# geoeo/ORB_SLAM3_V1.0

Hardware: AMD Instinct MI355X
Metric: frames/sec ORB extract+match, 752x480 8-level 1000-feat; bit-exact kp/desc (higher is better)
Workload: dtype u8

## Files before the change

### orb_slam3_v1.0_amd/csrc/kernels_match_proj.hip

```cpp
#include <algorithm>
#include <cstdio>
#include <cstdlib>
#include <cstring>

#include "device_math.h"
#include "match_common.h"

#include "match_proj.h"

#pragma clang fp contract(off)

namespace orbfe {

using namespace proj;

namespace {


template <bool LDS, class KeyFn>
__device__ __forceinline__ void block_sort_keys(unsigned long long* sKeys, unsigned long long* gKeys, int n, int P, int tid, KeyFn keyOf)
{
    for (int j = tid; j < P; j += 1024) {
        const unsigned long long key = j < n ? keyOf(j) : ~0ull;
        if constexpr (LDS) sKeys[j] = key;
        else gKeys[j] = key;
    }
    __syncthreads();
    for (int k2 = 2; k2 <= P; k2 <<= 1) {
        for (int j2 = k2 >> 1; j2 > 0; j2 >>= 1) {
            for (int t = tid; t < (P >> 1); t += 1024) {
                const int lo = ((t & ~(j2 - 1)) << 1) | (t & (j2 - 1));
                const int hi = lo | j2;
                const bool up = (lo & k2) == 0;
                unsigned long long a, b;
                if constexpr (LDS) { a = sKeys[lo]; b = sKeys[hi]; }
                else { a = gKeys[lo]; b = gKeys[hi]; }
                if ((a > b) == up) {
                    if constexpr (LDS) { sKeys[lo] = b; sKeys[hi] = a; }
                    else { gKeys[lo] = b; gKeys[hi] = a; }
                }
            }
            __syncthreads();
        }
    }
}

template <class KeyFn>
__device__ __forceinline__ void block_sort_keys_reg(unsigned long long* sKeys, int n, int P, int tid, KeyFn keyOf)
{
    unsigned long long key = tid < n ? keyOf(tid) : ~0ull;
    int buf = 0;
    for (int k2 = 2; k2 <= P; k2 <<= 1) {
        for (int j2 = k2 >> 1; j2 > 0; j2 >>= 1) {
            unsigned long long other;
            if (j2 >= 64) {
                unsigned long long* b = sKeys + buf * 1024;
                b[tid] = key;
                __syncthreads();
                other = b[tid ^ j2];
                buf ^= 1;
            } else {
                other = shfl_xor_u64(key, j2);
            }
            const bool up = (tid & k2) == 0;
            const bool lower = (tid & j2) == 0;
            const unsigned long long mn = key < other ? key : other, mx = key < other ? other : key;
            key = (lower == up) ? mn : mx;
        }
    }
    __syncthreads();
    sKeys[tid] = key;
    __syncthreads();
}

constexpr int kCellBits = 22;

template <bool LDS>
__device__ __forceinline__ void proj_grid_body(const ProjArgs& A)
{
    __shared__ unsigned long long sKeys[LDS ? kSortLds : 1];
    __shared__ int sRankOf[LDS ? kSortLds : 1];
    const int f = blockIdx.x;
    const int tid = threadIdx.x;
    const int n = min(A.nKp[f], A.kpStride);
    const int nCells = A.g.cols * A.g.rows;
    const orbfe_keypoint* kp = A.kp + (size_t)f * A.kpStride;
    unsigned long long* gKeys = A.sortKeys + (size_t)f * A.sortCap;
    int* gRankOf = A.rankOf + (size_t)f * A.kpStride;
    int P = 1;
    while (P < n) P <<= 1;
    for (int j = tid; j < A.kpStride; j += 1024) A.matchOut[(size_t)f * A.kpStride + j] = -1;
    auto cellOf = [&](int j) {
        const orbfe_keypoint& k = kp[j];
        float px = k.x - A.g.minX;
        px = px * A.g.invW;
        float py = k.y - A.g.minY;
        py = py * A.g.invH;
        const int posX = (int)roundf(px), posY = (int)roundf(py);
        const int lin = posY * A.g.cols + posX;
        int v = nCells;
        if (lin >= 0 && lin < nCells) v = (lin % A.g.cols) * A.g.rows + lin / A.g.cols;
        return v;
    };
    auto key1 = [&](int j) { return ((unsigned long long)cellOf(j) << kRankBits) | (unsigned long long)j; };
    const bool regSort = LDS && P <= 1024;
    if (regSort) block_sort_keys_reg(sKeys, n, P, tid, key1);
    else block_sort_keys<LDS>(sKeys, gKeys, n, P, tid, key1);
    for (int r = tid; r < n; r += 1024) {
        unsigned long long key;
        if constexpr (LDS) key = sKeys[r];
        else key = gKeys[r];
        const int idx = (int)(key & kRankMask);
        A.order[(size_t)f * A.kpStride + r] = idx;
        A.octByRank[(size_t)f * A.kpStride + r] = (uint8_t)min(max(kp[idx].octave, 0), 31);
        if constexpr (LDS) sRankOf[idx] = r;
        else gRankOf[idx] = r;
    }
    __syncthreads();
    auto key2 = [&](int j) {
        const unsigned long long lvl = (unsigned long long)min(max(kp[j].octave, 0), 31);
        return (lvl << (kRankBits + kCellBits + 1)) | ((unsigned long long)cellOf(j) << kRankBits) | (unsigned long long)j;
    };
    if (regSort) block_sort_keys_reg(sKeys, n, P, tid, key2);
    else block_sort_keys<LDS>(sKeys, gKeys, n, P, tid, key2);
    const unsigned long long* desc = reinterpret_cast<const unsigned long long*>(A.desc + (size_t)f * A.kpStride * 32);
    for (int p = tid; p < n; p += 1024) {
        unsigned long long key;
        if constexpr (LDS) key = sKeys[p];
        else key = gKeys[p];
        const int idx = (int)(key & kRankMask);
        const int v = (int)((key >> kRankBits) & ((1u << (kCellBits + 1)) - 1u));
        const int lvl = (int)(key >> (kRankBits + kCellBits + 1));
        const orbfe_keypoint k = kp[idx];
        int rank;
        if constexpr (LDS) rank = sRankOf[idx];
        else rank = gRankOf[idx];
        const int cy = v < nCells ? v % A.g.rows : 0x7fff;
        A.rec[(size_t)f * A.kpStride + p] = make_int4(rank, lvl | (cy << 8), __float_as_int(k.x), __float_as_int(k.y));
        unsigned long long* dd = A.descS + ((size_t)f * A.kpStride + p) * 4;
        dd[0] = desc[(size_t)idx * 4 + 0];
        dd[1] = desc[(size_t)idx * 4 + 1];
        dd[2] = desc[(size_t)idx * 4 + 2];
        dd[3] = desc[(size_t)idx * 4 + 3];
    }
    const int tabStride = A.g.cols + 1;
    int* cs = A.colStart + (size_t)f * A.tabLevels * tabStride;
    const int nTab = A.tabLevels * tabStride;
    for (int e = tid; e < nTab; e += 1024) {
        const int l = e / tabStride;
        const int v = (e - l * tabStride) * A.g.rows;
        const unsigned long long want = ((unsigned long long)l << (kCellBits + 1)) | (unsigned long long)v;
        int lo = 0, hi = n;
        while (lo < hi) {
            const int mid = (lo + hi) >> 1;
            unsigned long long key;
            if constexpr (LDS) key = sKeys[mid];
            else key = gKeys[mid];
            if ((key >> kRankBits) < want) lo = mid + 1;
            else hi = mid;
        }
        cs[e] = lo;
    }
}

constexpr int kTilesX = 8, kTilesY = 6;
constexpr int kSortBuckets = 32 * kTilesX * kTilesY + 1;

__device__ __forceinline__ int sort_bucket(const ProjArgs& A, const orbfe_map_point& mp)
{
    const bool valid = mp.in_view && !(A.farPoints && mp.track_depth > A.thFar) && !mp.bad;
    if (!valid) return kSortBuckets - 1;
    const int lvl = min(max(mp.level, 0), 31);
    const int cx = (int)((mp.proj_x - A.g.minX) * A.g.invW), cy = (int)((mp.proj_y - A.g.minY) * A.g.invH);
    const int tx = min(max(cx * kTilesX / A.g.cols, 0), kTilesX - 1);
    const int ty = min(max(cy * kTilesY / A.g.rows, 0), kTilesY - 1);
    return (lvl * kTilesY + ty) * kTilesX + tx;
}

__device__ __forceinline__ void proj_sort_body(const ProjArgs& A)
{
    __shared__ int sHist[kSortBuckets];
    const int f = blockIdx.x;
    const int tid = threadIdx.x;
    for (int b = tid; b < kSortBuckets; b += 1024) sHist[b] = 0;
    __syncthreads();
    const orbfe_map_point* mps = A.mps + (size_t)f * A.M;
    for (int i = tid; i < A.M; i += 1024) atomicAdd(&sHist[sort_bucket(A, mps[i])], 1);
    __syncthreads();
    {
        static_assert(kSortBuckets <= 2048, "two buckets per thread");
        __shared__ int sWaveTot[16];
        const int b0 = 2 * tid, b1 = 2 * tid + 1;
        const int c0 = b0 < kSortBuckets ? sHist[b0] : 0, c1 = b1 < kSortBuckets ? sHist[b1] : 0;
        const int lane = tid & 63, wv = tid >> 6;
        int incl = c0 + c1;
#pragma unroll
        for (int d = 1; d < 64; d <<= 1) {
            const int o = __shfl_up(incl, d);
            if (lane >= d) incl += o;
        }
        if (lane == 63) sWaveTot[wv] = incl;
        __syncthreads();
        int base = incl - (c0 + c1);
        for (int q = 0; q < wv; q++) base += sWaveTot[q];
        if (b0 < kSortBuckets) sHist[b0] = base;
        if (b1 < kSortBuckets) sHist[b1] = base + c0;
    }
    __syncthreads();
    for (int i = tid; i < A.M; i += 1024) {
        const int pos = atomicAdd(&sHist[sort_bucket(A, mps[i])], 1);
        A.perm[(size_t)f * A.M + pos] = i;
    }
}

template <bool LDS, bool SORT_MPS>
__global__ __launch_bounds__(1024) void proj_prepare_kernel(ProjArgs A)
{
    if constexpr (SORT_MPS) {
        if (blockIdx.y == 1) {
            proj_sort_body(A);
            return;
        }
    }
    proj_grid_body<LDS>(A);
}

constexpr int kTopkLds = 768;

struct TopkLds {
    int4 rec[kTopkLds];
    unsigned long long desc[kTopkLds][4];
};

template <bool LDS, bool WIDE>
__device__ __forceinline__ int topk_scan(const ProjArgs& A, const MpWindow& w, const int* cs, int tabStride, const int4* rec,
                                         const unsigned long long* descS, const TopkLds* S, int segBase,
                                         unsigned long long d0, unsigned long long d1, unsigned long long d2,
                                         unsigned long long d3, uint32_t (&keys)[kTopK])
{
    int total = 0;
    const int lFirst = max(w.minLevel, 0), l1 = w.maxLevel;
    for (int l0 = lFirst; l0 <= (WIDE ? l1 : lFirst); l0 += 2) {
    int plo[2], phi[2];
#pragma unroll
    for (int k = 0; k < 2; k++) {
        const int l = min(l0 + k, l1);
        const int* csl = cs + (size_t)l * tabStride;
        plo[k] = csl[w.minCX];
        phi[k] = (l0 + k <= l1) ? csl[w.maxCX + 1] : plo[k];
    }
#pragma unroll
    for (int k = 0; k < 2; k++) {
        int4 qn = make_int4(0, 0, 0, 0);
        if (plo[k] < phi[k]) {
            if constexpr (LDS) qn = S->rec[plo[k] - segBase];
            else qn = rec[plo[k]];
        }
        for (int p = plo[k]; p < phi[k]; p++) {
            const int4 q = qn;
            if (p + 1 < phi[k]) {
                if constexpr (LDS) qn = S->rec[p + 1 - segBase];
                else qn = rec[p + 1];
            }
            const int cy = q.y >> 8;
            if (cy < w.minCY || cy > w.maxCY) continue;
            const float dx = __int_as_float(q.z) - w.x, dy = __int_as_float(q.w) - w.y;
            if (!(fabsf(dx) < w.r && fabsf(dy) < w.r)) continue;
            int dist;
            if constexpr (LDS) {
                const unsigned long long* kd = S->desc[p - segBase];
                dist = __popcll(kd[0] ^ d0) + __popcll(kd[1] ^ d1) + __popcll(kd[2] ^ d2) + __popcll(kd[3] ^ d3);
            } else {
                const unsigned long long* kd = descS + (size_t)p * 4;
                dist = __popcll(kd[0] ^ d0) + __popcll(kd[1] ^ d1) + __popcll(kd[2] ^ d2) + __popcll(kd[3] ^ d3);
            }
            if (dist >= A.dCut) continue;
            total++;
            uint32_t key = make_key32(dist, q.x);
            if (key < keys[kTopK - 1]) {
#pragma unroll
                for (int t = kTopK - 1; t > 0; t--) keys[t] = umed3(keys[t - 1], key, keys[t]);
                keys[0] = min(keys[0], key);
            }
        }
    }
    }
    return total;
}

template <bool WIDE>
__global__ __launch_bounds__(256) void proj_topk_kernel(ProjArgs A)
{
    __shared__ TopkLds S;
    __shared__ int sLvlLo, sLvlHi;
    const int f = blockIdx.y;
    const int slotIdx = blockIdx.x * 256 + threadIdx.x;
    const bool live = slotIdx < A.M;
    const int i = live ? A.perm[(size_t)f * A.M + slotIdx] : 0;
    MpWindow w;
    w.valid = false;
    w.minLevel = w.maxLevel = 0;
    if (live) w = mp_window(A, A.mps[(size_t)f * A.M + i]);
    if (threadIdx.x == 0) { sLvlLo = 64; sLvlHi = -1; }
    __syncthreads();
    if (w.valid) {
        atomicMin(&sLvlLo, max(w.minLevel, 0));
        atomicMax(&sLvlHi, w.maxLevel);
    }
    __syncthreads();
    const int tabStride = A.g.cols + 1;
    const int* cs = A.colStart + (size_t)f * A.tabLevels * tabStride;
    const int4* rec = A.rec + (size_t)f * A.kpStride;
    const unsigned long long* descS = A.descS + (size_t)f * A.kpStride * 4;
    int segBase = 0, segEnd = 0;
    if (sLvlHi >= 0) {
        segBase = cs[(size_t)sLvlLo * tabStride];
        segEnd = sLvlHi + 1 < A.tabLevels ? cs[(size_t)(sLvlHi + 1) * tabStride] : min(A.nKp[f], A.kpStride);
    }
    const bool useLds = segEnd - segBase <= kTopkLds;
    if (useLds) {
        const int nSeg = segEnd - segBase;
        const uint4* gRec = reinterpret_cast<const uint4*>(rec + segBase);
        const uint4* gDesc = reinterpret_cast<const uint4*>(descS + (size_t)segBase * 4);
        uint4* lRec = reinterpret_cast<uint4*>(S.rec);
        uint4* lDesc = reinterpret_cast<uint4*>(&S.desc[0][0]);
        for (int j0 = 0; j0 < nSeg * 2; j0 += 4 * 256) {
            uint4 v[4];
#pragma unroll
            for (int k = 0; k < 4; k++) {
                const int j = j0 + k * 256 + (int)threadIdx.x;
                if (j < nSeg * 2) v[k] = gDesc[j];
            }
#pragma unroll
            for (int k = 0; k < 4; k++) {
                const int j = j0 + k * 256 + (int)threadIdx.x;
                if (j < nSeg * 2) lDesc[j] = v[k];
            }
        }
        for (int j0 = 0; j0 < nSeg; j0 += 4 * 256) {
            uint4 v[4];
#pragma unroll
            for (int k = 0; k < 4; k++) {
                const int j = j0 + k * 256 + (int)threadIdx.x;
                if (j < nSeg) v[k] = gRec[j];
            }
#pragma unroll
            for (int k = 0; k < 4; k++) {
                const int j = j0 + k * 256 + (int)threadIdx.x;
                if (j < nSeg) lRec[j] = v[k];
            }
        }
    }
    __syncthreads();
    if (!live) return;
    uint32_t keys[kTopK];
#pragma unroll
    for (int t = 0; t < kTopK; t++) keys[t] = kKey32None;
    int total = 0;
    if (w.valid) {
        const unsigned long long* dp = reinterpret_cast<const unsigned long long*>(A.mpDesc + ((size_t)f * A.M + i) * 32);
        const unsigned long long d0 = dp[0], d1 = dp[1], d2 = dp[2], d3 = dp[3];
        if (useLds) total = topk_scan<true, WIDE>(A, w, cs, tabStride, rec, descS, &S, segBase, d0, d1, d2, d3, keys);
        else total = topk_scan<false, WIDE>(A, w, cs, tabStride, rec, descS, &S, segBase, d0, d1, d2, d3, keys);
    }
    A.cnt[(size_t)f * A.M + i] = total;
    uint4* dst = reinterpret_cast<uint4*>(A.topk + ((size_t)f * A.M + i) * kTopK);
#pragma unroll
    for (int t = 0; t < kTopK / 4; t++) dst[t] = make_uint4(keys[4 * t], keys[4 * t + 1], keys[4 * t + 2], keys[4 * t + 3]);
}

constexpr int kWaveListCap = 128;

__device__ __forceinline__ void rank_emit_lds(const uint32_t* list, int n, int limit, uint32_t* out, int lane)
{
    const uint32_t e0 = lane < n ? list[lane] : kKey32None;
    const uint32_t e1 = lane + 64 < n ? list[lane + 64] : kKey32None;
    int r0 = 0, r1 = 0;
    for (int b = 0; b < n; b++) {
        const uint32_t kb = list[b];
        r0 += kb < e0;
        r1 += kb < e1;
    }
    __builtin_amdgcn_wave_barrier();
    if (lane < n && r0 < limit) out[r0] = e0;
    if (lane + 64 < n && r1 < limit) out[r1] = e1;
    asm volatile("s_waitcnt lgkmcnt(0)" ::: "memory");
    __builtin_amdgcn_wave_barrier();
}

template <bool WIDE, bool LDS>
__device__ __forceinline__ void topk_wave_body(const ProjArgs& A, const TopkLds& S, uint32_t (*sList)[2][kWaveListCap], int f, int lane,
                                               int wv, int nMine, int i, const MpWindow& w, const int* cs, int tabStride,
                                               const int4* rec, const unsigned long long* descS, int segBase)
{
    constexpr int NLV = WIDE ? 3 : 2;
    int plo[NLV], phi[NLV];
    {
        const int l0 = max(w.minLevel, 0), l1 = w.maxLevel;
#pragma unroll
        for (int k = 0; k < NLV; k++) {
            const int l = min(l0 + k, l1);
            const int* csl = cs + (size_t)l * tabStride;
            plo[k] = w.valid ? csl[w.minCX] : 0;
            phi[k] = (w.valid && l0 + k <= l1) ? csl[w.maxCX + 1] : plo[k];
        }
    }
    const int validI = w.valid ? 1 : 0;
    uint32_t dq[8] = {0, 0, 0, 0, 0, 0, 0, 0};
    if (w.valid) {
        const uint4* dp = reinterpret_cast<const uint4*>(A.mpDesc + ((size_t)f * A.M + i) * 32);
        const uint4 a = dp[0], b = dp[1];
        dq[0] = a.x; dq[1] = a.y; dq[2] = a.z; dq[3] = a.w; dq[4] = b.x; dq[5] = b.y; dq[6] = b.z; dq[7] = b.w;
    }
#pragma unroll
    for (int k = 0; k < NLV; k++) asm volatile("" : "+v"(plo[k]), "+v"(phi[k]));
#pragma unroll
    for (int k = 0; k < 8; k++) asm volatile("" : "+v"(dq[k]));
    {
        int iv = i;
        asm volatile("s_waitcnt vmcnt(0)" : "+v"(iv));
    }
    for (int j = 0; j < nMine; j++) {
        const int mp = __builtin_amdgcn_readlane(i, j);
        uint32_t* dst = A.topk + ((size_t)f * A.M + mp) * kTopK;
        int total = 0, listN = 0, cur = 0;
        if (__builtin_amdgcn_readlane(validI, j)) {
            const float x = __int_as_float(__builtin_amdgcn_readlane(__float_as_int(w.x), j));
            const float y = __int_as_float(__builtin_amdgcn_readlane(__float_as_int(w.y), j));
            const float r = __int_as_float(__builtin_amdgcn_readlane(__float_as_int(w.r), j));
            const int minCY = __builtin_amdgcn_readlane(w.minCY, j), maxCY = __builtin_amdgcn_readlane(w.maxCY, j);
            unsigned long long d[4];
#pragma unroll
            for (int k = 0; k < 4; k++)
                d[k] = (unsigned long long)(uint32_t)__builtin_amdgcn_readlane((int)dq[2 * k], j) |
                       ((unsigned long long)(uint32_t)__builtin_amdgcn_readlane((int)dq[2 * k + 1], j) << 32);
            int a[NLV], len[NLV], lenAll = 0;
#pragma unroll
            for (int k = 0; k < NLV; k++) {
                a[k] = __builtin_amdgcn_readlane(plo[k], j);
                len[k] = __builtin_amdgcn_readlane(phi[k], j) - a[k];
                lenAll += len[k];
            }
            for (int base = 0; base < lenAll; base += 64) {
                if (listN > 64) {
                    rank_emit_lds(sList[wv][cur], listN, 64, sList[wv][cur ^ 1], lane);
                    cur ^= 1;
                    listN = 64;
                }
                const int idx = base + lane;
                bool q = false;
                uint32_t key = kKey32None;
                if (idx < lenAll) {
                    int p = a[0] + idx;
                    if (idx >= len[0]) p = a[1] + (idx - len[0]);
                    if constexpr (NLV == 3)
                        if (idx >= len[0] + len[1]) p = a[2] + (idx - len[0] - len[1]);
                    int4 rq;
                    if constexpr (LDS) rq = S.rec[p - segBase];
                    else rq = rec[p];
                    const int cy = rq.y >> 8;
                    const float dx = __int_as_float(rq.z) - x, dy = __int_as_float(rq.w) - y;
                    if (cy >= minCY && cy <= maxCY && fabsf(dx) < r && fabsf(dy) < r) {
                        int dist;
                        if constexpr (LDS) {
                            const unsigned long long* kd = S.desc[p - segBase];
                            dist = __popcll(kd[0] ^ d[0]) + __popcll(kd[1] ^ d[1]) + __popcll(kd[2] ^ d[2]) + __popcll(kd[3] ^ d[3]);
                        } else {
                            const unsigned long long* kd = descS + (size_t)p * 4;
                            dist = __popcll(kd[0] ^ d[0]) + __popcll(kd[1] ^ d[1]) + __popcll(kd[2] ^ d[2]) + __popcll(kd[3] ^ d[3]);
                        }
                        if (dist < A.dCut) {
                            q = true;
                            key = make_key32(dist, rq.x);
                        }
                    }
                }
                const unsigned long long mask = __ballot(q);
                if (mask) {
                    if (q)
                        sList[wv][cur][listN + (int)__builtin_amdgcn_mbcnt_hi((uint32_t)(mask >> 32),
                                                                              __builtin_amdgcn_mbcnt_lo((uint32_t)mask, 0u))] = key;
                    const int c = __popcll(mask);
                    listN += c;
                    total += c;
                }
            }
            if (total) {
                asm volatile("s_waitcnt lgkmcnt(0)" ::: "memory");
                __builtin_amdgcn_wave_barrier();
                if (listN > 64) {
                    rank_emit_lds(sList[wv][cur], listN, 64, sList[wv][cur ^ 1], lane);
                    cur ^= 1;
                    listN = 64;
                }
                const uint32_t e = lane < listN ? sList[wv][cur][lane] : kKey32None;
                int rk = 0;
                for (int b = 0; b < listN; b++) rk += (uint32_t)__builtin_amdgcn_readlane((int)e, b) < e;
                if (lane < listN && rk < kTopK) dst[rk] = e;
                if (lane >= listN && lane < kTopK) dst[lane] = kKey32None;
            }
        }
        if (lane == 0) A.cnt[(size_t)f * A.M + mp] = total;
    }
}

template <bool WIDE>
__global__ __launch_bounds__(256) void proj_topk_wave_kernel(ProjArgs A, int mpw)
{
    __shared__ TopkLds S;
    __shared__ int sLvlLo, sLvlHi;
    __shared__ uint32_t sList[4][2][kWaveListCap];
    const int f = blockIdx.y;
    const int lane = threadIdx.x & 63;
    const int wv = __builtin_amdgcn_readfirstlane((int)(threadIdx.x >> 6));
    const int waveBase = (blockIdx.x * 4 + wv) * mpw;
    const int nMine = min(mpw, A.M - waveBase);
    const bool live = lane < nMine;
    const int i = live ? A.perm[(size_t)f * A.M + waveBase + lane] : 0;
    MpWindow w;
    w.valid = false;
    w.minLevel = w.maxLevel = 0;
    w.x = w.y = w.r = 0.0f;
    w.minCX = w.maxCX = w.minCY = w.maxCY = 0;
    if (live) w = mp_window(A, A.mps[(size_t)f * A.M + i]);
    if (threadIdx.x == 0) { sLvlLo = 64; sLvlHi = -1; }
    __syncthreads();
    if (w.valid) {
        atomicMin(&sLvlLo, max(w.minLevel, 0));
        atomicMax(&sLvlHi, w.maxLevel);
    }
    __syncthreads();
    const int tabStride = A.g.cols + 1;
    const int* cs = A.colStart + (size_t)f * A.tabLevels * tabStride;
    const int4* rec = A.rec + (size_t)f * A.kpStride;
    const unsigned long long* descS = A.descS + (size_t)f * A.kpStride * 4;
    int segBase = 0, segEnd = 0;
    if (sLvlHi >= 0) {
        segBase = cs[(size_t)sLvlLo * tabStride];
        segEnd = sLvlHi + 1 < A.tabLevels ? cs[(size_t)(sLvlHi + 1) * tabStride] : min(A.nKp[f], A.kpStride);
    }
    const bool useLds = segEnd - segBase <= kTopkLds;
    if (useLds) {
        const int nSeg = segEnd - segBase;
        const uint4* gRec = reinterpret_cast<const uint4*>(rec + segBase);
        const uint4* gDesc = reinterpret_cast<const uint4*>(descS + (size_t)segBase * 4);
        uint4* lRec = reinterpret_cast<uint4*>(S.rec);
        uint4* lDesc = reinterpret_cast<uint4*>(&S.desc[0][0]);
        for (int j0 = 0; j0 < nSeg * 2; j0 += 4 * 256) {
            uint4 v[4];
#pragma unroll
            for (int k = 0; k < 4; k++) {
                const int j = j0 + k * 256 + (int)threadIdx.x;
                if (j < nSeg * 2) v[k] = gDesc[j];
            }
#pragma unroll
            for (int k = 0; k < 4; k++) {
                const int j = j0 + k * 256 + (int)threadIdx.x;
                if (j < nSeg * 2) lDesc[j] = v[k];
            }
        }
        for (int j0 = 0; j0 < nSeg; j0 += 4 * 256) {
            uint4 v[4];
#pragma unroll
            for (int k = 0; k < 4; k++) {
                const int j = j0 + k * 256 + (int)threadIdx.x;
                if (j < nSeg) v[k] = gRec[j];
            }
#pragma unroll
            for (int k = 0; k < 4; k++) {
                const int j = j0 + k * 256 + (int)threadIdx.x;
                if (j < nSeg) lRec[j] = v[k];
            }
        }
    }
    __syncthreads();
    if (useLds) topk_wave_body<WIDE, true>(A, S, sList, f, lane, wv, nMine, i, w, cs, tabStride, rec, descS, segBase);
    else topk_wave_body<WIDE, false>(A, S, sList, f, lane, wv, nMine, i, w, cs, tabStride, rec, descS, segBase);
}

constexpr int kResN = 2048;

constexpr int kResNDesc = 1280;

template <int N, bool DESC>
struct ResolveLdsT {
    int claim[3][N];
    uint8_t oct[N];
    int4 rec[N];
    unsigned long long desc[DESC ? N * 4 : 4];
};

__device__ __forceinline__ void wave_top2_u32(uint32_t& k1, uint32_t& k2)
{
#pragma unroll
    for (int d = 32; d >= 1; d >>= 1) {
        const uint32_t o1 = __shfl_xor(k1, d), o2 = __shfl_xor(k2, d);
        const uint32_t lo = min(k1, o1), hi = max(k1, o1);
        k2 = min(hi, min(k2, o2));
        k1 = lo;
    }
}

template <bool LDS, bool DESC, typename SLds>
__device__ __forceinline__ void full_scan_top2_wave(const ProjArgs& A, int f, int i, const MpWindow& w,
                                                    const unsigned long long (&d4)[4], const int* cs, const int* claim,
                                                    const SLds* S, int lane, uint32_t& k1, uint32_t& k2)
{
    k1 = kKey32None;
    k2 = kKey32None;
    if (w.valid) {
        const int tabStride = A.g.cols + 1;
        const int4* rec = A.rec + (size_t)f * A.kpStride;
        const unsigned long long* descS = A.descS + (size_t)f * A.kpStride * 4;
        for (int l = max(w.minLevel, 0); l <= w.maxLevel; l++) {
            const int* csl = cs + (size_t)l * tabStride;
            const int plo = csl[w.minCX], phi = csl[w.maxCX + 1];
            for (int p = plo + lane; p < phi; p += 64) {
                int4 q;
                if constexpr (LDS) q = S->rec[p];
                else q = rec[p];
                if (claim[q.x] < i) continue;
                const int cy = q.y >> 8;
                if (cy < w.minCY || cy > w.maxCY) continue;
                const float dx = __int_as_float(q.z) - w.x, dy = __int_as_float(q.w) - w.y;
                if (!(fabsf(dx) < w.r && fabsf(dy) < w.r)) continue;
                int dist;
                if constexpr (DESC) dist = hamming256(reinterpret_cast<const uint2*>(S->desc + (size_t)p * 4), d4);
                else dist = hamming256(reinterpret_cast<const uint2*>(descS + (size_t)p * 4), d4);
                if (dist >= A.dCut) continue;
                const uint32_t key = make_key32(dist, q.x);
                if (key < k1) { k2 = k1; k1 = key; }
                else if (key < k2) k2 = key;
            }
        }
    }
    wave_top2_u32(k1, k2);
}

constexpr int kFbLds = 192;
constexpr int kResTabLds = 1024;

template <bool LDS, int THREADS, int N = kResN, bool DESC = false>
__global__ __launch_bounds__(THREADS) void proj_resolve_kernel(ProjArgs A)
{
    __shared__ ResolveLdsT<N, DESC> S;
    __shared__ int sChanged[2];
    __shared__ int sGaveUp[2];
    __shared__ int sCount;
    __shared__ int sFbCount[2];
    __shared__ int sFbMp[THREADS];
    __shared__ uint32_t sFbK1[THREADS], sFbK2[THREADS];
    __shared__ MpWindow sFbWin[kFbLds];
    __shared__ unsigned long long sFbDesc[kFbLds][4];
    __shared__ int sTab[LDS ? kResTabLds : 1];
    const int f = blockIdx.x;
    const int tid = threadIdx.x;
    const int n = min(A.nKp[f], A.kpStride);
    const int M = A.M;
    int* T[3];
#pragma unroll
    for (int q = 0; q < 3; q++) T[q] = LDS ? S.claim[q] : A.claimG + ((size_t)f * 3 + q) * A.kpStride;
    int fin = 0, cur = 1, nxt = 2;
    const orbfe_map_point* mps = A.mps + (size_t)f * M;
    const int* order = A.order + (size_t)f * A.kpStride;
    const int4* rec = A.rec + (size_t)f * A.kpStride;
    const int* initObs = A.initObs ? A.initObs + (size_t)f * A.kpStride : nullptr;

    for (int r = tid; r < n; r += THREADS) {
        const int v = (initObs && initObs[order[r]] > 0) ? -1 : kClaimFree;
        T[fin][r] = v;
        T[cur][r] = v;
    }
    const uint8_t* octByRank = A.octByRank + (size_t)f * A.kpStride;
    if constexpr (LDS) {
        for (int r = tid; r < n; r += THREADS) {
            S.rec[r] = rec[r];
            S.oct[r] = octByRank[r];
        }
    }
    if constexpr (DESC) {
        const unsigned long long* dsrc = A.descS + (size_t)f * A.kpStride * 4;
        for (int q = tid; q < n * 4; q += THREADS) S.desc[q] = dsrc[q];
    }
    const int tabStride = A.g.cols + 1;
    const int* csG = A.colStart + (size_t)f * A.tabLevels * tabStride;
    const bool tabInLds = LDS && A.tabLevels * tabStride <= kResTabLds;
    if (tabInLds)
        for (int k = tid; k < A.tabLevels * tabStride; k += THREADS) sTab[k] = csG[k];
    const int* cs = tabInLds ? sTab : csG;
    if (tid == 0) sCount = 0;
    int nAccepted = 0;
    __syncthreads();

    for (int chunk = 0; chunk < M; chunk += THREADS) {
        const int i = chunk + tid;
        const bool live = i < M;
        int c = 0, obs = 0;
        uint32_t keys[kTopK];
#pragma unroll
        for (int t = 0; t < kTopK; t++) keys[t] = kKey32None;
        if (live) {
            c = A.cnt[(size_t)f * M + i];
            obs = mps[i].observations;
            if (c > 0) {
                const uint4* src = reinterpret_cast<const uint4*>(A.topk + ((size_t)f * M + i) * kTopK);
#pragma unroll
                for (int t = 0; t < kTopK / 4; t++) {
                    const uint4 q = src[t];
                    keys[4 * t] = q.x; keys[4 * t + 1] = q.y; keys[4 * t + 2] = q.z; keys[4 * t + 3] = q.w;
                }
            }
        }
        int res = -1;
        uint32_t k1 = kKey32None, k2 = kKey32None;
        bool k2StandIn = false;
        for (int iter = 0; iter <= THREADS + 1; iter++) {
            if (tid == 0) { sChanged[iter & 1] = 0; sFbCount[iter & 1] = 0; sGaveUp[iter & 1] = 0; }
            if (res >= 0 && obs > 0) atomicMin(&T[cur][res], i);
            __syncthreads();
            const int* claim = T[cur];
            bool look = iter == 0 || sGaveUp[(iter & 1) ^ 1] != 0;
            if (!look && c > 0) {
                const int c1 = k1 != kKey32None ? claim[(int)(k1 & kRankMask)] : kClaimFree;
                const int c2 = (k2 != kKey32None && !k2StandIn) ? claim[(int)(k2 & kRankMask)] : kClaimFree;
                look = c1 < i || c2 < i;
            }
            int slot = -1;
            if (c > 0 && look) {
                k1 = kKey32None;
                k2 = kKey32None;
                k2StandIn = false;
                int cl[kTopK];
#pragma unroll
                for (int t = 0; t < kTopK; t++) cl[t] = claim[keys[t] != kKey32None ? (int)(keys[t] & kRankMask) : 0];
#pragma unroll
                for (int t = 0; t < kTopK; t++) {
                    const uint32_t m = cl[t] >= i ? keys[t] : kKey32None;
                    k2 = umed3(k1, m, k2);
                    k1 = min(k1, m);
                }
                if (k2 == kKey32None && c > kTopK) {
                    const int dK = (int)(keys[kTopK - 1] >> kRankBits);
                    bool decided = false;
                    if (k1 == kKey32None) decided = dK > ORBFE_TH_HIGH;
                    else {
                        const int bd = (int)(k1 >> kRankBits);
                        decided = bd > ORBFE_TH_HIGH || (A.nnRatio > 0.f && !((float)bd > A.nnRatio * (float)dK));
                        if (decided) {
                            k2 = keys[kTopK - 1];
                            k2StandIn = true;
                        }
                    }
                    if (!decided) {
                        slot = atomicAdd(&sFbCount[iter & 1], 1);
                        sFbMp[slot] = i;
                        if (slot < kFbLds) {
                            sFbWin[slot] = mp_window(A, mps[i]);
                            const unsigned long long* dp = reinterpret_cast<const unsigned long long*>(A.mpDesc + ((size_t)f * M + i) * 32);
#pragma unroll
                            for (int t = 0; t < 4; t++) sFbDesc[slot][t] = dp[t];
                        }
#ifdef ORBFE_DIAG
                        atomicAdd(&A.dbg[f * 4 + 1], 1);
#endif
                    }
                }
            }
            for (int k = tid; k < n; k += THREADS) T[nxt][k] = T[fin][k];
            auto verdict = [&]() {
                int result = -1;
                if (k1 != kKey32None) {
                    const int bestDist = (int)(k1 >> kRankBits), bestRank = (int)(k1 & kRankMask);
                    int bestLevel;
                    if constexpr (LDS) bestLevel = S.oct[bestRank];
                    else bestLevel = octByRank[bestRank];
                    int bestDist2 = 256, bestLevel2 = -1;
                    if (k2 != kKey32None) {
                        bestDist2 = (int)(k2 >> kRankBits);
                        const int r2 = (int)(k2 & kRankMask);
                        if constexpr (LDS) bestLevel2 = S.oct[r2];
                        else bestLevel2 = octByRank[r2];
                    }
                    if (bestDist <= ORBFE_TH_HIGH) {
                        const bool reject = bestLevel == bestLevel2 && (float)bestDist > A.nnRatio * (float)bestDist2;
                        if (!reject) result = bestRank;
                    }
                }
                return result;
            };
            auto move_to = [&](int result) {
                if (result != res) {
                    if (res >= 0 && obs > 0 && claim[res] == i) sGaveUp[iter & 1] = 1;
                    res = result;
                    sChanged[iter & 1] = 1;
                }
            };
            if (slot < 0 && look && c > 0) move_to(verdict());
            __syncthreads();
            if (sFbCount[iter & 1] > 0) {
                const int nFb = sFbCount[iter & 1];
                for (int q = __builtin_amdgcn_readfirstlane(tid >> 6); q < nFb; q += THREADS / 64) {
                    uint32_t a1, a2;
                    const int mp = sFbMp[q];
                    MpWindow w;
                    unsigned long long d4[4];
                    if (q < kFbLds) {
                        w = sFbWin[q];
#pragma unroll
                        for (int t = 0; t < 4; t++) d4[t] = sFbDesc[q][t];
                    } else {
                        w = mp_window(A, mps[mp]);
                        const unsigned long long* dp = reinterpret_cast<const unsigned long long*>(A.mpDesc + ((size_t)f * M + mp) * 32);
#pragma unroll
                        for (int t = 0; t < 4; t++) d4[t] = dp[t];
                    }
                    full_scan_top2_wave<LDS, DESC>(A, f, mp, w, d4, cs, claim, &S, tid & 63, a1, a2);
                    if ((tid & 63) == 0) { sFbK1[q] = a1; sFbK2[q] = a2; }
                }
                __syncthreads();
                if (slot >= 0) {
                    k1 = sFbK1[slot];
                    k2 = sFbK2[slot];
                    move_to(verdict());
                }
                __syncthreads();
            }
#ifdef ORBFE_DIAG
            if (tid == 0) atomicAdd(&A.dbg[f * 4 + 0], 1);
#endif
            if (!sChanged[iter & 1]) break;
            const int tq = cur;
            cur = nxt;
            nxt = tq;
        }
        {
            const int tq = fin;
            fin = cur;
            cur = tq;
        }
        if (chunk + THREADS < M) {
            for (int k = tid; k < n; k += THREADS) T[cur][k] = T[fin][k];
            __syncthreads();
        }
        if (res >= 0) {
            atomicMax(&A.matchOut[(size_t)f * A.kpStride + order[res]], i);
            nAccepted++;
        }
    }
    if (nAccepted) atomicAdd(&sCount, nAccepted);
    __syncthreads();
    if (tid == 0) A.nMatches[f] = sCount;
}

}

namespace proj {

void proj_prepare_launch(hipStream_t s, const ProjArgs& A, bool sortMps)
{
    const bool lds = A.kpStride <= kSortLds;
    if (sortMps) {
        if (lds) hipLaunchKernelGGL((proj_prepare_kernel<true, true>), dim3(A.B, 2), dim3(1024), 0, s, A);
        else hipLaunchKernelGGL((proj_prepare_kernel<false, true>), dim3(A.B, 2), dim3(1024), 0, s, A);
    } else {
        if (lds) hipLaunchKernelGGL((proj_prepare_kernel<true, false>), dim3(A.B), dim3(1024), 0, s, A);
        else hipLaunchKernelGGL((proj_prepare_kernel<false, false>), dim3(A.B), dim3(1024), 0, s, A);
    }
}

int proj_dcut(float nnRatio)
{
    int D = 256;
    for (int d = 0; d < 256; d++)
        if (!((float)ORBFE_TH_HIGH > nnRatio * (float)d)) {
            D = d;
            break;
        }
    return std::max(D, ORBFE_TH_HIGH + 1);
}

int proj_setup(MatchScratch& m, ProjArgs& A, Carver sc, size_t hostNeed, std::string& err, size_t* endOff)
{
    const int B = A.B, M = A.M;
    A.sortCap = 1;
    while (A.sortCap < A.kpStride) A.sortCap <<= 1;
    const bool ldsSort = A.kpStride <= kSortLds;
    const size_t oKeys = sc.take(ldsSort ? 8 : (size_t)B * A.sortCap * sizeof(unsigned long long));
    A.tabLevels = std::min(std::max(A.nLevels, 1), 32);
    A.dCut = proj_dcut(A.nnRatio);
    const size_t oOrder = sc.take((size_t)B * A.kpStride * sizeof(int));
    const size_t oOct = sc.take((size_t)B * A.kpStride);
    const size_t oRankOf = sc.take(ldsSort ? 8 : (size_t)B * A.kpStride * sizeof(int));
    const size_t oRec = sc.take((size_t)B * A.kpStride * sizeof(int4));
    const size_t oDescS = sc.take((size_t)B * A.kpStride * 32);
    const size_t oCol = sc.take((size_t)B * A.tabLevels * ((size_t)A.g.cols + 1) * sizeof(int));
    const size_t oCnt = sc.take((size_t)B * std::max(M, 1) * sizeof(int));
    const size_t oTopk = sc.take((size_t)B * kTopK * std::max(M, 1) * sizeof(uint32_t));
    const size_t oClaim = sc.take((size_t)B * 3 * A.kpStride * sizeof(int));
    const size_t oPerm = sc.take((size_t)B * std::max(M, 1) * sizeof(int));
    const size_t oDbg = sc.take((size_t)B * 4 * sizeof(int));
    if (endOff) *endOff = sc.off;
    int rc = ensure(m, sc.off, hostNeed + 256, err);
    if (rc != ORBFE_OK) return rc;
    uint8_t* dp = static_cast<uint8_t*>(m.d);
    A.sortKeys = reinterpret_cast<unsigned long long*>(dp + oKeys);
    A.order = reinterpret_cast<int*>(dp + oOrder);
    A.octByRank = dp + oOct;
    A.rankOf = reinterpret_cast<int*>(dp + oRankOf);
    A.rec = reinterpret_cast<int4*>(dp + oRec);
    A.descS = reinterpret_cast<unsigned long long*>(dp + oDescS);
    A.colStart = reinterpret_cast<int*>(dp + oCol);
    A.cnt = reinterpret_cast<int*>(dp + oCnt);
    A.topk = reinterpret_cast<uint32_t*>(dp + oTopk);
    A.claimG = reinterpret_cast<int*>(dp + oClaim);
    A.perm = reinterpret_cast<int*>(dp + oPerm);
    A.dbg = reinterpret_cast<int*>(dp + oDbg);
    return ORBFE_OK;
}

int proj_launch(hipStream_t s, ProjArgs& A, std::string& err)
{
    if (A.M == 0) {
        proj_prepare_launch(s, A, false);
        MCHK(hipMemsetAsync(A.nMatches, 0, (size_t)A.B * sizeof(int), s));
        return ORBFE_OK;
    }
#ifdef ORBFE_DIAG
    MCHK(hipMemsetAsync(A.dbg, 0, (size_t)A.B * 4 * sizeof(int), s));
#endif
    proj_prepare_launch(s, A, true);
    const int blocks256 = (A.M + 255) / 256;
    if ((long long)blocks256 * A.B >= 128) {
        if (A.mode == kModeReloc)
            hipLaunchKernelGGL(proj_topk_kernel<true>, dim3(blocks256, A.B), dim3(256), 0, s, A);
        else
            hipLaunchKernelGGL(proj_topk_kernel<false>, dim3(blocks256, A.B), dim3(256), 0, s, A);
    } else {
        int mpw = 64;
        while (mpw > 1 && (long long)((A.M + 4 * mpw - 1) / (4 * mpw)) * A.B < 512) mpw >>= 1;
        const dim3 grid((A.M + 4 * mpw - 1) / (4 * mpw), A.B);
        if (A.mode == kModeReloc)
            hipLaunchKernelGGL(proj_topk_wave_kernel<true>, grid, dim3(256), 0, s, A, mpw);
        else
            hipLaunchKernelGGL(proj_topk_wave_kernel<false>, grid, dim3(256), 0, s, A, mpw);
    }
    const bool lds = A.kpStride <= kResN;
#ifdef ORBFE_DIAG
    static const int envT = getenv("ORBFE_RESOLVE_THREADS") ? atoi(getenv("ORBFE_RESOLVE_THREADS")) : 0;
    const int rt = envT ? envT : kResolveThreads;
#else
    const int rt = kResolveThreads;
#endif
    if (lds && A.kpStride <= kResNDesc && rt == kResolveThreads) {
        hipLaunchKernelGGL((proj_resolve_kernel<true, kResolveThreads, kResNDesc, true>), dim3(A.B), dim3(kResolveThreads), 0, s, A);
    } else if (rt == 256) {
        if (lds) hipLaunchKernelGGL((proj_resolve_kernel<true, 256>), dim3(A.B), dim3(256), 0, s, A);
        else hipLaunchKernelGGL((proj_resolve_kernel<false, 256>), dim3(A.B), dim3(256), 0, s, A);
    } else {
        if (lds) hipLaunchKernelGGL((proj_resolve_kernel<true, kResolveThreads>), dim3(A.B), dim3(kResolveThreads), 0, s, A);
        else hipLaunchKernelGGL((proj_resolve_kernel<false, kResolveThreads>), dim3(A.B), dim3(kResolveThreads), 0, s, A);
    }
    MCHK(hipGetLastError());
    return ORBFE_OK;
}

}

void match_scratch_free(MatchScratch& m)
{
    if (m.d) (void)hipFree(m.d);
    if (m.hpin) (void)hipHostFree(m.hpin);
    m = MatchScratch();
}

int match_projection_run(MatchScratch& m, hipStream_t s, const orbfe_frame_view* F, int M, const orbfe_map_point* mps,
                         const uint8_t* mpDesc, const int* initObs, float th, int farPoints, float thFar,
                         float nnRatio, int* matchOut, int* nMatches, std::string& err)
{
    const int n = F->n;
    for (int i = 0; i < n; i++) matchOut[i] = -1;
    *nMatches = 0;
    if (n == 0 || M == 0) return ORBFE_OK;
    if (n >= (1 << 20) || F->grid_cols > 65535 || F->grid_rows > 32767 || F->n_levels < 1 ||
        (long long)F->grid_cols * F->grid_rows > kMaxCells)
        return ORBFE_ERR_UNSUPPORTED;
    for (int i = 0; i < M; i++)
        if (mps[i].in_view && (mps[i].level < 0 || mps[i].level >= F->n_levels)) return ORBFE_ERR_INVALID_ARG;

    Carver in;
    const size_t oKp = in.take((size_t)n * sizeof(orbfe_keypoint));
    const size_t oDesc = in.take((size_t)n * 32);
    const size_t oMp = in.take((size_t)M * sizeof(orbfe_map_point));
    const size_t oMpDesc = in.take((size_t)M * 32);
    const size_t oObs = in.take((size_t)n * sizeof(int));
    const size_t oSf = in.take((size_t)F->n_levels * sizeof(float));
    const size_t oN = in.take(sizeof(int));
    const size_t oMatch = in.take((size_t)n * sizeof(int));
    const size_t oNM = in.take(sizeof(int));
    const size_t inBytes = in.off;
    const size_t hostNeed = inBytes + (size_t)n * sizeof(int) + 64;

    ProjArgs A{};
    A.B = 1; A.M = M; A.kpStride = n;
    A.g = GridDesc{F->grid_cols, F->grid_rows, F->min_x, F->min_y, F->grid_inv_w, F->grid_inv_h};
    A.th = th; A.thFar = thFar; A.nnRatio = nnRatio; A.farPoints = farPoints; A.bFactor = th != 1.0;
    A.nLevels = F->n_levels;
    int rc = proj_setup(m, A, in, hostNeed, err);
    if (rc != ORBFE_OK) return rc;
    uint8_t* hp = static_cast<uint8_t*>(m.hpin);
    uint8_t* dp = static_cast<uint8_t*>(m.d);
    memcpy(hp + oKp, F->kp, (size_t)n * sizeof(orbfe_keypoint));
    memcpy(hp + oDesc, F->desc, (size_t)n * 32);
    memcpy(hp + oMp, mps, (size_t)M * sizeof(orbfe_map_point));
    memcpy(hp + oMpDesc, mpDesc, (size_t)M * 32);
    if (initObs) memcpy(hp + oObs, initObs, (size_t)n * sizeof(int));
    memcpy(hp + oSf, F->scale_factors, (size_t)F->n_levels * sizeof(float));
    memcpy(hp + oN, &n, sizeof(int));
    MCHK(hipMemcpyAsync(dp, hp, oMatch, hipMemcpyHostToDevice, s));
    A.kp = reinterpret_cast<const orbfe_keypoint*>(dp + oKp);
    A.desc = dp + oDesc;
    A.nKp = reinterpret_cast<const int*>(dp + oN);
    A.mps = reinterpret_cast<const orbfe_map_point*>(dp + oMp);
    A.mpDesc = dp + oMpDesc;
    A.initObs = initObs ? reinterpret_cast<const int*>(dp + oObs) : nullptr;
    A.scaleFactors = reinterpret_cast<const float*>(dp + oSf);
    A.matchOut = reinterpret_cast<int*>(dp + oMatch);
    A.nMatches = reinterpret_cast<int*>(dp + oNM);
    int* hNM = reinterpret_cast<int*>(hp + inBytes);
    int* hMatch = hNM + 2;
    rc = proj_launch(s, A, err);
    if (rc != ORBFE_OK) return rc;
    MCHK(hipMemcpyAsync(hMatch, A.matchOut, (size_t)n * sizeof(int), hipMemcpyDeviceToHost, s));
    MCHK(hipMemcpyAsync(hNM, A.nMatches, sizeof(int), hipMemcpyDeviceToHost, s));
    MCHK(hipStreamSynchronize(s));
#ifdef ORBFE_DIAG
    if (getenv("ORBFE_DEBUG_MATCH")) {
        int dbg[4] = {0, 0, 0, 0};
        (void)copy_sync(dbg, A.dbg, sizeof dbg, hipMemcpyDeviceToHost, s);
        fprintf(stderr, "[orbfe] match_projection: n=%d M=%d sweeps=%d cooperative_rescans=%d\n", n, M, dbg[0], dbg[1]);
    }
#endif
    memcpy(matchOut, hMatch, (size_t)n * sizeof(int));
    *nMatches = *hNM;
    return ORBFE_OK;
}

int match_projection_batch_device(MatchScratch& m, hipStream_t s, int B, const orbfe_keypoint* dKp, const uint8_t* dDesc,
                                  const int* dN, int kpStride, int gridCols, int gridRows, float minX, float minY,
                                  float invW, float invH, const float* dScaleFactors, int nLevels, int M,
                                  const orbfe_map_point* dMps, const uint8_t* dMpDesc, const int* dInitObs, float th,
                                  int farPoints, float thFar, float nnRatio, int* dMatchOut, int* dNMatches,
                                  std::string& err)
{
    if (kpStride >= (1 << 20) || gridCols > 65535 || gridRows > 32767 || (long long)gridCols * gridRows > kMaxCells)
        return ORBFE_ERR_UNSUPPORTED;
    ProjArgs A{};
    A.B = B; A.M = M; A.kpStride = kpStride;
    A.g = GridDesc{gridCols, gridRows, minX, minY, invW, invH};
    A.th = th; A.thFar = thFar; A.nnRatio = nnRatio; A.farPoints = farPoints; A.bFactor = th != 1.0;
    A.kp = dKp; A.desc = dDesc; A.nKp = dN; A.mps = dMps; A.mpDesc = dMpDesc; A.initObs = dInitObs;
    A.scaleFactors = dScaleFactors; A.nLevels = nLevels;
    A.matchOut = dMatchOut;
    A.nMatches = dNMatches;
    int rc = proj_setup(m, A, Carver(), 64, err);
    if (rc != ORBFE_OK) return rc;
    return proj_launch(s, A, err);
}

}
```

### orb_slam3_v1.0_amd/csrc/match_proj.h

```cpp
#pragma once
#include <string>

#include "match_common.h"

namespace orbfe {
namespace proj {

constexpr int kClaimFree = 0x7fffffff;
constexpr int kResolveThreads = 1024;
constexpr int kTopK = 24;
constexpr uint32_t kKey32None = 0xffffffffu;
constexpr int kRankBits = 20;
constexpr uint32_t kRankMask = (1u << kRankBits) - 1u;
constexpr int kSortLds = 2048;
constexpr int kMaxCells = 1 << 22;

struct GridDesc {
    int cols, rows;
    float minX, minY, invW, invH;
};

struct ProjArgs {
    int B, M, kpStride;
    GridDesc g;
    float th, thFar, nnRatio;
    int farPoints, bFactor;
    int mode;
    int dCut;
    const orbfe_keypoint* kp;
    const uint8_t* desc;
    const int* nKp;
    const orbfe_map_point* mps;
    const uint8_t* mpDesc;
    const int* initObs;
    const float* scaleFactors;
    int nLevels;
    int sortCap;
    unsigned long long* sortKeys;
    int* order;
    uint8_t* octByRank;
    int* rankOf;
    int4* rec;
    unsigned long long* descS;
    int* colStart;
    int tabLevels;
    int* cnt;
    uint32_t* topk;
    int* claimG;
    int* perm;
    int* dbg;
    int* matchOut;
    int* nMatches;
};

constexpr int kModeReloc = 1;

struct MpWindow {
    bool valid;
    float x, y, r;
    int minCX, maxCX, minCY, maxCY, minLevel, maxLevel;
};

__device__ __forceinline__ void window_cells(const GridDesc& g, MpWindow& w);

__device__ __forceinline__ MpWindow mp_window(const ProjArgs& A, const orbfe_map_point& mp)
{
    MpWindow w;
    w.valid = mp.in_view && !(A.farPoints && mp.track_depth > A.thFar) && !mp.bad;
    const int lvl = w.valid ? min(max(mp.level, 0), A.nLevels - 1) : 0;
    float r;
    if (A.mode == kModeReloc) r = A.th * A.scaleFactors[lvl];
    else {
        r = mp.view_cos > 0.998 ? 2.5f : 4.0f;
        if (A.bFactor) r = r * A.th;
        r = r * A.scaleFactors[lvl];
    }
    w.r = r;
    w.x = mp.proj_x;
    w.y = mp.proj_y;
    window_cells(A.g, w);
    w.minLevel = lvl - 1;
    w.maxLevel = A.mode == kModeReloc ? min(lvl + 1, A.nLevels - 1) : lvl;
    return w;
}

__device__ __forceinline__ void window_cells(const GridDesc& g, MpWindow& w)
{
    const float r = w.r;
    float t;
    t = w.x - g.minX; t = t - r; t = t * g.invW;
    w.minCX = max(0, (int)floorf(t));
    t = w.x - g.minX; t = t + r; t = t * g.invW;
    w.maxCX = min(g.cols - 1, (int)ceilf(t));
    t = w.y - g.minY; t = t - r; t = t * g.invH;
    w.minCY = max(0, (int)floorf(t));
    t = w.y - g.minY; t = t + r; t = t * g.invH;
    w.maxCY = min(g.rows - 1, (int)ceilf(t));
    if (w.minCX >= g.cols || w.maxCX < 0 || w.minCY >= g.rows || w.maxCY < 0) w.valid = false;
}

__device__ __forceinline__ uint32_t umed3(uint32_t a, uint32_t b, uint32_t c) { return max(min(a, b), min(max(a, b), c)); }

__device__ __forceinline__ uint32_t make_key32(int dist, int rank) { return ((uint32_t)dist << kRankBits) | (uint32_t)rank; }

int proj_dcut(float nnRatio);
int proj_setup(MatchScratch& m, ProjArgs& A, Carver sc, size_t hostNeed, std::string& err, size_t* endOff = nullptr);
void proj_prepare_launch(hipStream_t s, const ProjArgs& A, bool sortMps);
int proj_launch(hipStream_t s, ProjArgs& A, std::string& err);

}
}
```

Baseline: 210,900.

## Add lean 256-thread resolve kernel variant for large frame batches

When the batch holds many frames, the resolve kernel now launches a 256-thread variant without the LDS keypoint-record image and with a smaller fallback window buffer. This cuts LDS use per block so more blocks fit per CU across many frames. The claim-table indices are replaced by direct pointers, and the top-2 update in the fallback scan becomes a branchless med3/min. The trade-off is fewer threads per frame and more global reads of records and octaves, with more fallback rescans spilling past the LDS buffer.

```diff
diff --git a/orb_slam3_v1.0_amd/csrc/kernels_match_proj.hip b/orb_slam3_v1.0_amd/csrc/kernels_match_proj.hip
--- a/orb_slam3_v1.0_amd/csrc/kernels_match_proj.hip
+++ b/orb_slam3_v1.0_amd/csrc/kernels_match_proj.hip
@@ -582,11 +582,11 @@
 
 constexpr int kResNDesc = 1280;
 
-template <int N, bool DESC>
+template <int N, bool DESC, bool IMG>
 struct ResolveLdsT {
     int claim[3][N];
-    uint8_t oct[N];
-    int4 rec[N];
+    uint8_t oct[IMG ? N : 1];
+    int4 rec[IMG ? N : 1];
     unsigned long long desc[DESC ? N * 4 : 4];
 };
 
@@ -601,7 +601,7 @@
     }
 }
 
-template <bool LDS, bool DESC, typename SLds>
+template <bool IMG, bool DESC, typename SLds>
 __device__ __forceinline__ void full_scan_top2_wave(const ProjArgs& A, int f, int i, const MpWindow& w,
                                                     const unsigned long long (&d4)[4], const int* cs, const int* claim,
                                                     const SLds* S, int lane, uint32_t& k1, uint32_t& k2)
@@ -617,7 +617,7 @@
             const int plo = csl[w.minCX], phi = csl[w.maxCX + 1];
             for (int p = plo + lane; p < phi; p += 64) {
                 int4 q;
-                if constexpr (LDS) q = S->rec[p];
+                if constexpr (IMG) q = S->rec[p];
                 else q = rec[p];
                 if (claim[q.x] < i) continue;
                 const int cy = q.y >> 8;
@@ -629,8 +629,8 @@
                 else dist = hamming256(reinterpret_cast<const uint2*>(descS + (size_t)p * 4), d4);
                 if (dist >= A.dCut) continue;
                 const uint32_t key = make_key32(dist, q.x);
-                if (key < k1) { k2 = k1; k1 = key; }
-                else if (key < k2) k2 = key;
+                k2 = umed3(k1, key, k2);
+                k1 = min(k1, key);
             }
         }
     }
@@ -639,28 +639,29 @@
 
 constexpr int kFbLds = 192;
 constexpr int kResTabLds = 1024;
-
-template <bool LDS, int THREADS, int N = kResN, bool DESC = false>
+constexpr int kFbBatched = 32;
+
+template <bool LDS, int THREADS, int N = kResN, bool DESC = false, bool IMG = LDS, int FB = kFbLds>
 __global__ __launch_bounds__(THREADS) void proj_resolve_kernel(ProjArgs A)
 {
-    __shared__ ResolveLdsT<N, DESC> S;
+    static_assert(LDS || !IMG, "the LDS image goes with LDS claim tables");
+    __shared__ ResolveLdsT<N, DESC, IMG> S;
     __shared__ int sChanged[2];
     __shared__ int sGaveUp[2];
     __shared__ int sCount;
     __shared__ int sFbCount[2];
     __shared__ int sFbMp[THREADS];
     __shared__ uint32_t sFbK1[THREADS], sFbK2[THREADS];
-    __shared__ MpWindow sFbWin[kFbLds];
-    __shared__ unsigned long long sFbDesc[kFbLds][4];
+    __shared__ MpWindow sFbWin[FB];
+    __shared__ unsigned long long sFbDesc[FB][4];
     __shared__ int sTab[LDS ? kResTabLds : 1];
     const int f = blockIdx.x;
     const int tid = threadIdx.x;
     const int n = min(A.nKp[f], A.kpStride);
     const int M = A.M;
-    int* T[3];
-#pragma unroll
-    for (int q = 0; q < 3; q++) T[q] = LDS ? S.claim[q] : A.claimG + ((size_t)f * 3 + q) * A.kpStride;
-    int fin = 0, cur = 1, nxt = 2;
+    int* Tfin = LDS ? S.claim[0] : A.claimG + ((size_t)f * 3 + 0) * A.kpStride;
+    int* Tcur = LDS ? S.claim[1] : A.claimG + ((size_t)f * 3 + 1) * A.kpStride;
+    int* Tnxt = LDS ? S.claim[2] : A.claimG + ((size_t)f * 3 + 2) * A.kpStride;
     const orbfe_map_point* mps = A.mps + (size_t)f * M;
     const int* order = A.order + (size_t)f * A.kpStride;
     const int4* rec = A.rec + (size_t)f * A.kpStride;
@@ -668,11 +669,11 @@
 
     for (int r = tid; r < n; r += THREADS) {
         const int v = (initObs && initObs[order[r]] > 0) ? -1 : kClaimFree;
-        T[fin][r] = v;
-        T[cur][r] = v;
+        Tfin[r] = v;
+        Tcur[r] = v;
     }
     const uint8_t* octByRank = A.octByRank + (size_t)f * A.kpStride;
-    if constexpr (LDS) {
+    if constexpr (IMG) {
         for (int r = tid; r < n; r += THREADS) {
             S.rec[r] = rec[r];
             S.oct[r] = octByRank[r];
@@ -716,9 +717,9 @@
         bool k2StandIn = false;
         for (int iter = 0; iter <= THREADS + 1; iter++) {
             if (tid == 0) { sChanged[iter & 1] = 0; sFbCount[iter & 1] = 0; sGaveUp[iter & 1] = 0; }
-            if (res >= 0 && obs > 0) atomicMin(&T[cur][res], i);
+            if (res >= 0 && obs > 0) atomicMin(&Tcur[res], i);
             __syncthreads();
-            const int* claim = T[cur];
+            const int* claim = Tcur;
             bool look = iter == 0 || sGaveUp[(iter & 1) ^ 1] != 0;
             if (!look && c > 0) {
                 const int c1 = k1 != kKey32None ? claim[(int)(k1 & kRankMask)] : kClaimFree;
@@ -754,7 +755,7 @@
                     if (!decided) {
                         slot = atomicAdd(&sFbCount[iter & 1], 1);
                         sFbMp[slot] = i;
-                        if (slot < kFbLds) {
+                        if (slot < FB) {
                             sFbWin[slot] = mp_window(A, mps[i]);
                             const unsigned long long* dp = reinterpret_cast<const unsigned long long*>(A.mpDesc + ((size_t)f * M + i) * 32);
 #pragma unroll
@@ -762,23 +763,24 @@
                         }
 #ifdef ORBFE_DIAG
                         atomicAdd(&A.dbg[f * 4 + 1], 1);
+                        if (slot >= FB) atomicAdd(&A.dbg[f * 4 + 2], 1);
 #endif
                     }
                 }
             }
-            for (int k = tid; k < n; k += THREADS) T[nxt][k] = T[fin][k];
+            for (int k = tid; k < n; k += THREADS) Tnxt[k] = Tfin[k];
             auto verdict = [&]() {
                 int result = -1;
                 if (k1 != kKey32None) {
                     const int bestDist = (int)(k1 >> kRankBits), bestRank = (int)(k1 & kRankMask);
                     int bestLevel;
-                    if constexpr (LDS) bestLevel = S.oct[bestRank];
+                    if constexpr (IMG) bestLevel = S.oct[bestRank];
                     else bestLevel = octByRank[bestRank];
                     int bestDist2 = 256, bestLevel2 = -1;
                     if (k2 != kKey32None) {
                         bestDist2 = (int)(k2 >> kRankBits);
                         const int r2 = (int)(k2 & kRankMask);
-                        if constexpr (LDS) bestLevel2 = S.oct[r2];
+                        if constexpr (IMG) bestLevel2 = S.oct[r2];
                         else bestLevel2 = octByRank[r2];
                     }
                     if (bestDist <= ORBFE_TH_HIGH) {
@@ -804,7 +806,7 @@
                     const int mp = sFbMp[q];
                     MpWindow w;
                     unsigned long long d4[4];
-                    if (q < kFbLds) {
+                    if (q < FB) {
                         w = sFbWin[q];
 #pragma unroll
                         for (int t = 0; t < 4; t++) d4[t] = sFbDesc[q][t];
@@ -814,7 +816,7 @@
 #pragma unroll
                         for (int t = 0; t < 4; t++) d4[t] = dp[t];
                     }
-                    full_scan_top2_wave<LDS, DESC>(A, f, mp, w, d4, cs, claim, &S, tid & 63, a1, a2);
+                    full_scan_top2_wave<IMG, DESC>(A, f, mp, w, d4, cs, claim, &S, tid & 63, a1, a2);
                     if ((tid & 63) == 0) { sFbK1[q] = a1; sFbK2[q] = a2; }
                 }
                 __syncthreads();
@@ -829,17 +831,17 @@
             if (tid == 0) atomicAdd(&A.dbg[f * 4 + 0], 1);
 #endif
             if (!sChanged[iter & 1]) break;
-            const int tq = cur;
-            cur = nxt;
-            nxt = tq;
+            int* const tq = Tcur;
+            Tcur = Tnxt;
+            Tnxt = tq;
         }
         {
-            const int tq = fin;
-            fin = cur;
-            cur = tq;
+            int* const tq = Tfin;
+            Tfin = Tcur;
+            Tcur = tq;
         }
         if (chunk + THREADS < M) {
-            for (int k = tid; k < n; k += THREADS) T[cur][k] = T[fin][k];
+            for (int k = tid; k < n; k += THREADS) Tcur[k] = Tfin[k];
             __syncthreads();
         }
         if (res >= 0) {
@@ -945,13 +947,17 @@
             hipLaunchKernelGGL(proj_topk_wave_kernel<false>, grid, dim3(256), 0, s, A, mpw);
     }
     const bool lds = A.kpStride <= kResN;
+    const bool batched = A.B >= kResolveBatchedMinFrames;
 #ifdef ORBFE_DIAG
-    static const int envT = getenv("ORBFE_RESOLVE_THREADS") ? atoi(getenv("ORBFE_RESOLVE_THREADS")) : 0;
-    const int rt = envT ? envT : kResolveThreads;
+    static const int envT = getenv("ORBFE_RESOLVE_THREADS") ? atoi(getenv("ORBFE_RESOLVE_THREADS")) : -1;
+    const int rt = envT >= 0 ? envT : (batched ? 0 : kResolveThreads);
 #else
-    const int rt = kResolveThreads;
+    const int rt = batched ? 0 : kResolveThreads;
 #endif
-    if (lds && A.kpStride <= kResNDesc && rt == kResolveThreads) {
+    if (rt == 0) {
+        if (lds) hipLaunchKernelGGL((proj_resolve_kernel<true, 256, kResN, false, false, kFbBatched>), dim3(A.B), dim3(256), 0, s, A);
+        else hipLaunchKernelGGL((proj_resolve_kernel<false, 256, kResN, false, false, kFbBatched>), dim3(A.B), dim3(256), 0, s, A);
+    } else if (lds && A.kpStride <= kResNDesc && rt == kResolveThreads) {
         hipLaunchKernelGGL((proj_resolve_kernel<true, kResolveThreads, kResNDesc, true>), dim3(A.B), dim3(kResolveThreads), 0, s, A);
     } else if (rt == 256) {
         if (lds) hipLaunchKernelGGL((proj_resolve_kernel<true, 256>), dim3(A.B), dim3(256), 0, s, A);
@@ -1037,7 +1043,8 @@
     if (getenv("ORBFE_DEBUG_MATCH")) {
         int dbg[4] = {0, 0, 0, 0};
         (void)copy_sync(dbg, A.dbg, sizeof dbg, hipMemcpyDeviceToHost, s);
-        fprintf(stderr, "[orbfe] match_projection: n=%d M=%d sweeps=%d cooperative_rescans=%d\n", n, M, dbg[0], dbg[1]);
+        fprintf(stderr, "[orbfe] match_projection: n=%d M=%d sweeps=%d cooperative_rescans=%d unparked_rescans=%d\n", n, M, dbg[0], dbg[1],
+                dbg[2]);
     }
 #endif
     memcpy(matchOut, hMatch, (size_t)n * sizeof(int));
diff --git a/orb_slam3_v1.0_amd/csrc/match_proj.h b/orb_slam3_v1.0_amd/csrc/match_proj.h
--- a/orb_slam3_v1.0_amd/csrc/match_proj.h
+++ b/orb_slam3_v1.0_amd/csrc/match_proj.h
@@ -8,6 +8,7 @@
 
 constexpr int kClaimFree = 0x7fffffff;
 constexpr int kResolveThreads = 1024;
+constexpr int kResolveBatchedMinFrames = 384;
 constexpr int kTopK = 24;
 constexpr uint32_t kKey32None = 0xffffffffu;
 constexpr int kRankBits = 20;
```

New measurement: 221,000, median of 6. 4.8% higher.
